# researchaccelerator-hub/distributed-crawler

Measured on AMD Instinct MI355X. Metric: posts/sec (whole node) synthetic feed, higher is better.
Workload: dtype uint8; 1 GPU; model=telegram-crawl 1k-channels x 10k-posts per GPU (BASELINE config #2, weak-scaled), global_batch=1250000, seq_len=0, platform=telegram, parallelism=dp1, channels_per_gpu=1000, posts_per_channel=10000, chunk_posts=1250000, new_discoveries=998486, sink=pinned, pinned=True, max_comments_per_post=3

## Files before the change

crawler_amd/ops/csrc/parse_encode.hip:

```cpp

#include "common.h"
#include "tg_lits.h"

namespace crawl {

#define MAX_LINKS 8
#define TG_STAGE_BYTES 3968

struct BatchView {
  const long* __restrict__ chat_id;
  const long* __restrict__ msg_id;
  const long* __restrict__ text_off;
  const int* __restrict__ date;
  const int* __restrict__ content_type;
  const int* __restrict__ views;
  const int* __restrict__ forwards;
  const int* __restrict__ media_album_id;
  const int* __restrict__ channel_idx;
  const int* __restrict__ flags;
  const int* __restrict__ text_len;
  const int* __restrict__ aux_off;
  const int* __restrict__ aux_len;
  const int* __restrict__ ent_off;
  const int* __restrict__ ent_cnt;
  const int* __restrict__ react_off;
  const int* __restrict__ react_cnt;
  const int* __restrict__ com_off;
  const int* __restrict__ com_cnt;
  const int* __restrict__ poster_off;
  const int* __restrict__ poster_len;
  const unsigned char* __restrict__ pool;
  const int* __restrict__ entities;
  const int* __restrict__ react_emoji;
  const int* __restrict__ react_count;
  const int* __restrict__ com_text_off;
  const int* __restrict__ com_text_len;
  const int* __restrict__ com_handle_off;
  const int* __restrict__ com_handle_len;
  const int* __restrict__ com_views;
  const int* __restrict__ com_replies;
  const int* __restrict__ com_react_off;
  const int* __restrict__ com_react_cnt;
  const long* __restrict__ ch_chat_id;
  const int* __restrict__ ch_member;
  const int* __restrict__ ch_postcount;
  const int* __restrict__ ch_totalviews;
  const int* __restrict__ ch_user_off;
  const int* __restrict__ ch_user_len;
  const int* __restrict__ ch_title_off;
  const int* __restrict__ ch_title_len;
  const unsigned char* __restrict__ emoji_pool;
  const int* __restrict__ emoji_off;
  const int* __restrict__ emoji_len;
  const unsigned char* __restrict__ created_str;
  int created_len;
  const unsigned char* __restrict__ capture_str;
  int capture_len;
  int n;
  int skip_media;
  long min_post_date;
  const unsigned char* __restrict__ ctname_pool;
  const int* __restrict__ ctname_off;
  const int* __restrict__ ctname_len;
};

struct LinkOut {
  unsigned char* __restrict__ name;
  unsigned char* __restrict__ name_len;
  unsigned char* __restrict__ src;
  int* __restrict__ cnt;
  unsigned long long* __restrict__ hash;
};


DEV void utf16_to_bytes(const unsigned char* s, int n, int off16, int len16,
                        int* out_start, int* out_end) {
  int lane = lane_id();
  int run = 0;
  int start = -1, end = -1;
  const int t1 = off16, t2 = off16 + len16;
  for (int base = 0; base < n; base += WAVE) {
    int p = base + lane;
    int u = (p < n) ? u16_units_of_byte(s[p]) : 0;
    int pre = run + wave_prefix_excl(u);
    bool boundary = (p < n) && u > 0;
    unsigned long long m1 = __ballot(boundary && pre == t1);
    unsigned long long m2 = __ballot(boundary && pre == t2);
    if (start < 0 && m1) start = base + __ffsll(m1) - 1;
    if (end < 0 && m2) end = base + __ffsll(m2) - 1;
    run += wave_sum(u);
    if (end >= 0) break;
  }
  if (start < 0) { *out_start = 0; *out_end = 0; return; }
  *out_start = start;
  *out_end = (end >= 0) ? end : n;
}


DEV bool is_reserved_path(const unsigned char* name, int n) {
  const char* tbl[10] = {"joinchat", "addlist", "addstickers", "addtheme",
                         "setlanguage", "share", "proxy", "socks", "login",
                         "confirm"};
  const int lens[10] = {8, 7, 11, 8, 11, 5, 5, 5, 5, 7};
  for (int k = 0; k < 10; ++k) {
    if (lens[k] != n) continue;
    bool eq = true;
    for (int j = 0; j < n; ++j) eq &= (name[j] == (unsigned char)tbl[k][j]);
    if (eq) return true;
  }
  return false;
}

DEV int match_name_at(const unsigned char* s, int hi, int q,
                      unsigned char* name, bool* reserved) {
  *reserved = false;
  if (q >= hi || !is_ascii_letter(s[q])) return 0;
  int len = 0;
  while (len < 32 && q + len < hi && is_word_char(s[q + len])) ++len;
  if (len < 5) return 0;
  for (int j = 0; j < len; ++j) name[j] = to_lower(s[q + j]);
  *reserved = is_reserved_path(name, len);
  return len;
}

DEV int find_tme(const unsigned char* s, int from, int hi, int lane) {
  for (int base = from; base + 5 <= hi; base += WAVE) {
    int p = base + lane;
    bool m = (p + 5 <= hi) && s[p] == 't' && s[p + 1] == '.' &&
             s[p + 2] == 'm' && s[p + 3] == 'e' && s[p + 4] == '/';
    unsigned long long bal = __ballot(m);
    if (bal) return base + __ffsll(bal) - 1;
  }
  return -1;
}

DEV int find_username(const unsigned char* s, int lo, int hi, int lane,
                      unsigned char* name) {
  for (int base = lo; base < hi; base += WAVE) {
    int p = base + lane;
    bool m = false;
    if (p < hi && p + 5 <= hi && is_ascii_letter(s[p])) {
      m = is_word_char(s[p + 1]) && is_word_char(s[p + 2]) &&
          is_word_char(s[p + 3]) && is_word_char(s[p + 4]);
    }
    unsigned long long bal = __ballot(m);
    if (bal) {
      int q = base + __ffsll(bal) - 1;
      int len = 0;
      while (len < 32 && q + len < hi && is_word_char(s[q + len])) ++len;
      for (int j = 0; j < len; ++j) name[j] = to_lower(s[q + j]);
      return len;
    }
  }
  return 0;
}

struct LinkList {
  unsigned char* names;
  unsigned char* lens;
  unsigned char* srcs;
  unsigned long long* hashes;
  int cnt;

  DEV void add(const unsigned char* name, int len, int src, int lane) {
    for (int k = 0; k < cnt; ++k) {
      if (lens[k] != (unsigned char)len) continue;
      bool eq = true;
      for (int j = 0; j < len; ++j) eq &= (names[k * 32 + j] == name[j]);
      if (eq) return;
    }
    if (cnt >= MAX_LINKS) return;
    if (lane == 0) {
      for (int j = 0; j < len; ++j) names[cnt * 32 + j] = name[j];
      lens[cnt] = (unsigned char)len;
      srcs[cnt] = (unsigned char)src;
      hashes[cnt] = fnv1a64(name, len);
    }
    ++cnt;
  }
};

DEV void extract_links(const BatchView& B, int i, LinkList& L, int lane) {
  int ct = B.content_type[i];
  if (ct > 6) return;
  const unsigned char* text = B.pool + B.text_off[i];
  const int tn = B.text_len[i];
  unsigned char name[32];

  const int e0 = B.ent_off[i], ec = B.ent_cnt[i];
  for (int e = e0; e < e0 + ec; ++e) {
    const int* row = B.entities + (long)e * 5;
    int etype = row[0];
    if (etype == 1) {
      const unsigned char* url = B.pool + row[3];
      int un = row[4];
      for (int from = 0;;) {
        int p = find_tme(url, from, un, lane);
        if (p < 0) break;
        bool rsv;
        int len = match_name_at(url, un, p + 5, name, &rsv);
        if (len) {
          if (!rsv) L.add(name, len, 1, lane);
          break;
        }
        from = p + 1;
      }
    } else {
      int lo, hi;
      utf16_to_bytes(text, tn, row[1], row[2], &lo, &hi);
      if (!(lo < hi && hi <= tn)) continue;
      if (etype == 0) {
        int len = find_username(text, lo, hi, lane, name);
        if (len) L.add(name, len, 0, lane);
      } else {
        for (int from = lo;;) {
          int p = find_tme(text, from, hi, lane);
          if (p < 0) break;
          bool rsv;
          int len = match_name_at(text, hi, p + 5, name, &rsv);
          if (len) {
            if (!rsv) L.add(name, len, 2, lane);
            break;
          }
          from = p + 1;
        }
      }
    }
  }

  int cursor = 0;
  int from = 0;
  while (true) {
    int p = find_tme(text, from, tn, lane);
    if (p < 0) break;
    from = p + 1;
    if (p < cursor) continue;
    bool rsv;
    int len = match_name_at(text, tn, p + 5, name, &rsv);
    if (len) {
      if (!rsv) L.add(name, len, 3, lane);
      cursor = p + 5 + len;
      from = cursor;
    }
  }
}


template <bool W>
struct Emit : JsonEmit<W> {
  DEV void qesc(const unsigned char* s, int n) {
    LIT(*this, "\"");
    this->esc(s, n);
    LIT(*this, "\"");
  }
};

struct StagedTabs {
  const unsigned char* emoji_pool;
  const int* emoji_off;
  const int* emoji_len;
  const unsigned char* created;
  const unsigned char* capture;
  const unsigned char* ctname_pool;
  const int* ctname_off;
  const int* ctname_len;
};

template <bool W, bool STAGED>
DEV int emit_line(const BatchView& B, int i, unsigned char* out,
                  LinkList& L, const unsigned char* lds_lits,
                  unsigned char* lds_stage, const StagedTabs* T) {
  const int lane = lane_id();
  Emit<W> e{};
  e.out = out;
  e.cur = 0;
  e.lds = lds_lits;
  const int c = B.channel_idx[i];
  const unsigned char* user = B.pool + B.ch_user_off[c];
  const int user_n = B.ch_user_len[c];
  const unsigned char* title = B.pool + B.ch_title_off[c];
  const int title_n = B.ch_title_len[c];
  const long pub_id = B.msg_id[i] >> 20;
  const int ct = B.content_type[i];
  const int ncom = B.com_cnt[i];
  const bool has_user = user_n > 0;
  const long chat_id_v = B.chat_id[i];
  const int media_album = B.media_album_id[i];
  const int date_v = B.date[i];
  const int views_v = B.views[i];
  const int forwards_v = B.forwards[i];
  const int ch_member_v = B.ch_member[c];
  const int ch_postcount_v = B.ch_postcount[c];
  const int ch_totalviews_v = B.ch_totalviews[c];
  const int flags_v = B.flags[i];
  const int com0_v = B.com_off[i];
  const int react0_v = B.react_off[i];
  const int reactc_v = B.react_cnt[i];
  const int poster_off_v = B.poster_off[i];
  const int poster_len_v = B.poster_len[i];
  const int text_off_v = B.text_off[i];
  const int text_len_v = B.text_len[i];
  const int aux_off_v = B.aux_off[i];
  const int aux_len_v = B.aux_len[i];
  const int ctname_off_v = B.ctname_off[ct];
  const int ctname_len_v = B.ctname_len[ct];
  const unsigned char* desc_p;
  int desc_n;
  if (ct == 0 || ct == 1 || ct == 2 || ct == 4 || ct == 14) {
    desc_p = B.pool + text_off_v;
    desc_n = text_len_v;
  } else if (ct == 3 || ct == 9 || ct == 10 || ct == 11) {
    desc_p = B.pool + aux_off_v;
    desc_n = aux_len_v;
  } else {
    desc_p = nullptr;
    desc_n = 0;
  }
  const unsigned char* poster_p = B.pool + poster_off_v;
  const int* re_src = B.react_emoji + react0_v;
  const int* rcnt_src = B.react_count + react0_v;
  const unsigned char* lnames_src = L.names;
  const unsigned char* llens_src = L.lens;
  if (STAGED) {
    int stage_o = 0;
    auto staged = [&](const unsigned char* ptr,
                      int n) -> const unsigned char* {
      unsigned char* dst = lds_stage + stage_o;
      stage_o += n;
      for (int j = lane; j < n; j += WAVE) dst[j] = ptr[j];
      return dst;
    };
    user = staged(user, user_n);
    title = staged(title, title_n);
    poster_p = staged(poster_p, poster_len_v);
    desc_p = staged(desc_p, desc_n);
    lnames_src = staged(L.names, L.cnt * 32);
    llens_src = staged(L.lens, L.cnt);
    stage_o = (stage_o + 3) & ~3;
    int* s_re = (int*)(lds_stage + stage_o);
    stage_o += reactc_v * 4;
    int* s_rc = (int*)(lds_stage + stage_o);
    stage_o += reactc_v * 4;
    for (int j = lane; j < reactc_v; j += WAVE) {
      s_re[j] = B.react_emoji[react0_v + j];
      s_rc[j] = B.react_count[react0_v + j];
    }
    re_src = s_re;
    rcnt_src = s_rc;
  }
  const unsigned char* emoji_pool_s = STAGED ? T->emoji_pool : B.emoji_pool;
  const int* emoji_off_s = STAGED ? T->emoji_off : B.emoji_off;
  const int* emoji_len_s = STAGED ? T->emoji_len : B.emoji_len;
  const unsigned char* created_s = STAGED ? T->created : B.created_str;
  const unsigned char* capture_s = STAGED ? T->capture : B.capture_str;
  const unsigned char* ctpool_s = STAGED ? T->ctname_pool : B.ctname_pool;

  auto post_link = [&]() {
    if (!has_user) { LIT(e, "\"\""); return; }
    TGLIT(e, TGL_0);
    e.esc(user, user_n);
    LIT(e, "/");
    e.i64(pub_id);
    if (media_album != 0) TGLIT(e, TGL_1);
    LIT(e, "\"");
  };

  TGLIT(e, TGL_2);
  post_link();
  TGLIT(e, TGL_3);
  e.i64(chat_id_v);
  TGLIT(e, TGL_4);
  e.i64(pub_id);
  LIT(e, "-");
  e.esc(user, user_n);
  TGLIT(e, TGL_5);
  post_link();
  TGLIT(e, TGL_6);
  e.rfc3339(date_v);
  TGLIT(e, TGL_7);
  e.raw(created_s, B.created_len);
  TGLIT(e, TGL_8);
  e.i64(views_v);
  TGLIT(e, TGL_9);
  e.i64(views_v);
  TGLIT(e, TGL_10);
  e.i64(forwards_v);
  TGLIT(e, TGL_11);
  e.i64(ncom);
  TGLIT(e, TGL_12);
  e.qesc(title, title_n);
  TGLIT(e, TGL_13);
  e.i64(chat_id_v);
  TGLIT(e, TGL_14);
  e.qesc(title, title_n);
  TGLIT(e, TGL_15);
  e.i64(ch_member_v);
  TGLIT(e, TGL_16);
  e.i64(ch_postcount_v);
  TGLIT(e, TGL_17);
  e.i64(ch_totalviews_v);
  TGLIT(e, TGL_18);
  e.esc(user, user_n);
  TGLIT(e, TGL_19);
  e.esc(user, user_n);
  TGLIT(e, TGL_20);
  e.qesc(desc_p, desc_n);
  TGLIT(e, TGL_21);
  e.raw(ctpool_s + (STAGED ? T->ctname_off[ct] : ctname_off_v),
        STAGED ? T->ctname_len[ct] : ctname_len_v);
  TGLIT(e, TGL_22);
  e.i64(forwards_v);
  TGLIT(e, TGL_23);
  e.i64(ncom);
  TGLIT(e, TGL_17);
  e.i64(views_v);
  TGLIT(e, TGL_24);
  TGLIT(e, TGL_25);
  if ((ct == 3 || ct == 8) && (flags_v & 2)) {
    LIT(e, "AgAD");
    e.i64(pub_id);
    LIT(e, "v");
  }
  TGLIT(e, TGL_26);
  {
    const int c0 = com0_v;
    for (int k = 0; k < ncom; ++k) {
      if (k) LIT(e, ",");
      const int cc = c0 + k;
      TGLIT(e, TGL_27);
      e.qesc(B.pool + B.com_text_off[cc], B.com_text_len[cc]);
      TGLIT(e, TGL_28);
      const int r0 = B.com_react_off[cc], rc = B.com_react_cnt[cc];
      for (int r = 0; r < rc; ++r) {
        if (r) LIT(e, ",");
        int em = B.react_emoji[r0 + r];
        LIT(e, "\"");
        e.raw(emoji_pool_s + emoji_off_s[em], emoji_len_s[em]);
        LIT(e, "\":");
        e.i64(B.react_count[r0 + r]);
      }
      TGLIT(e, TGL_29);
      e.i64(B.com_views[cc]);
      TGLIT(e, TGL_30);
      e.i64(B.com_replies[cc]);
      TGLIT(e, TGL_31);
      e.qesc(B.pool + B.com_handle_off[cc], B.com_handle_len[cc]);
      LIT(e, "}");
    }
  }
  TGLIT(e, TGL_32);
  {
    const int rc = reactc_v;
    for (int r = 0; r < rc; ++r) {
      if (r) LIT(e, ",");
      int em = re_src[r];
      LIT(e, "\"");
      e.raw(emoji_pool_s + emoji_off_s[em], emoji_len_s[em]);
      LIT(e, "\":");
      e.i64(rcnt_src[r]);
    }
  }
  TGLIT(e, TGL_33);
  for (int k = 0; k < L.cnt; ++k) {
    if (k) LIT(e, ",");
    LIT(e, "\"");
    e.raw(lnames_src + k * 32, llens_src[k]);
    LIT(e, "\"");
  }
  TGLIT(e, TGL_34);
  e.raw(capture_s, B.capture_len);
  TGLIT(e, TGL_35);
  e.qesc(poster_p, poster_len_v);
  LIT(e, "}\n");
  return e.cur;
}


__global__ void __launch_bounds__(256, 6)
measure_extract_kernel(BatchView B, LinkOut LO, int* __restrict__ line_len) {
  __shared__ unsigned char s_lits[TG_POOL_BYTES];
  __shared__ unsigned char s_ln[4][MAX_LINKS * 32];
  __shared__ unsigned char s_ll[4][MAX_LINKS];
  __shared__ unsigned char s_ls[4][MAX_LINKS];
  __shared__ unsigned long long s_lh[4][MAX_LINKS];
  for (int t = threadIdx.x; t < TG_POOL_BYTES; t += blockDim.x)
    s_lits[t] = (unsigned char)tg_lit_pool.v[t];
  __syncthreads();
  const int lane = lane_id();
  const int wave = wave_id();
  const int waves_per_grid = gridDim.x * 4;
  for (int i = blockIdx.x * 4 + wave; i < B.n; i += waves_per_grid) {
    if ((long)B.date[i] < B.min_post_date) {
      if (lane == 0) { line_len[i] = 0; LO.cnt[i] = 0; }
      continue;
    }
    LinkList L{&s_ln[wave][0], &s_ll[wave][0], &s_ls[wave][0],
               &s_lh[wave][0], 0};
    extract_links(B, i, L, lane);
    int len = emit_line<false, false>(B, i, nullptr, L, s_lits,
                                     nullptr, nullptr);
    const int nb = L.cnt * 32;
    unsigned char* gname = LO.name + (size_t)i * MAX_LINKS * 32;
    for (int j = lane; j < nb; j += WAVE) gname[j] = s_ln[wave][j];
    if (lane < L.cnt) {
      LO.name_len[(size_t)i * MAX_LINKS + lane] = s_ll[wave][lane];
      LO.src[(size_t)i * MAX_LINKS + lane] = s_ls[wave][lane];
      LO.hash[(size_t)i * MAX_LINKS + lane] = s_lh[wave][lane];
    }
    if (lane == 0) {
      line_len[i] = len;
      LO.cnt[i] = L.cnt;
    }
  }
}

__global__ void __launch_bounds__(256, 4)
write_kernel(BatchView B, LinkOut LO, const long* __restrict__ line_off,
             const int* __restrict__ line_len, unsigned char* __restrict__ out) {
  __shared__ unsigned char s_lits[TG_POOL_BYTES];
  for (int t = threadIdx.x; t < TG_POOL_BYTES; t += blockDim.x)
    s_lits[t] = (unsigned char)tg_lit_pool.v[t];
  __syncthreads();
  const int lane = lane_id();
  const int wave = wave_id();
  const int waves_per_grid = gridDim.x * 4;
  for (int i = blockIdx.x * 4 + wave; i < B.n; i += waves_per_grid) {
    if (line_len[i] == 0) continue;
    LinkList L{LO.name + (size_t)i * MAX_LINKS * 32,
               LO.name_len + (size_t)i * MAX_LINKS,
               LO.src + (size_t)i * MAX_LINKS,
               LO.hash + (size_t)i * MAX_LINKS, LO.cnt[i]};
    emit_line<true, false>(B, i, out + line_off[i], L, s_lits, nullptr,
                           nullptr);
  }
}

#define TG_EMOJI_POOL_CAP 512
#define TG_EMOJI_CAP 64
#define TG_TS_CAP 64
#define TG_CTNAME_POOL_CAP 512
#define TG_CTNAME_CAP 32

__global__ void __launch_bounds__(256, 4)
write_staged_kernel(BatchView B, LinkOut LO, const long* __restrict__ line_off,
                    const int* __restrict__ line_len,
                    unsigned char* __restrict__ out,
                    int n_emoji, int emoji_pool_bytes,
                    int n_ctnames, int ctname_pool_bytes) {
  __shared__ unsigned char s_lits[TG_POOL_BYTES];
  __shared__ unsigned char s_stage[4][TG_STAGE_BYTES];
  __shared__ unsigned char s_emoji_pool[TG_EMOJI_POOL_CAP];
  __shared__ int s_emoji_off[TG_EMOJI_CAP];
  __shared__ int s_emoji_len[TG_EMOJI_CAP];
  __shared__ unsigned char s_created[TG_TS_CAP];
  __shared__ unsigned char s_capture[TG_TS_CAP];
  __shared__ unsigned char s_ctpool[TG_CTNAME_POOL_CAP];
  __shared__ int s_ctoff[TG_CTNAME_CAP];
  __shared__ int s_ctlen[TG_CTNAME_CAP];
  for (int t = threadIdx.x; t < TG_POOL_BYTES; t += blockDim.x)
    s_lits[t] = (unsigned char)tg_lit_pool.v[t];
  for (int t = threadIdx.x; t < emoji_pool_bytes; t += blockDim.x)
    s_emoji_pool[t] = B.emoji_pool[t];
  for (int t = threadIdx.x; t < n_emoji; t += blockDim.x) {
    s_emoji_off[t] = B.emoji_off[t];
    s_emoji_len[t] = B.emoji_len[t];
  }
  for (int t = threadIdx.x; t < B.created_len; t += blockDim.x)
    s_created[t] = B.created_str[t];
  for (int t = threadIdx.x; t < B.capture_len; t += blockDim.x)
    s_capture[t] = B.capture_str[t];
  for (int t = threadIdx.x; t < ctname_pool_bytes; t += blockDim.x)
    s_ctpool[t] = B.ctname_pool[t];
  for (int t = threadIdx.x; t < n_ctnames; t += blockDim.x) {
    s_ctoff[t] = B.ctname_off[t];
    s_ctlen[t] = B.ctname_len[t];
  }
  __syncthreads();
  StagedTabs T{s_emoji_pool, s_emoji_off, s_emoji_len, s_created,
               s_capture, s_ctpool, s_ctoff, s_ctlen};
  const int lane = lane_id();
  const int wave = wave_id();
  const int waves_per_grid = gridDim.x * 4;
  for (int i = blockIdx.x * 4 + wave; i < B.n; i += waves_per_grid) {
    if (line_len[i] == 0) continue;
    LinkList L{LO.name + (size_t)i * MAX_LINKS * 32,
               LO.name_len + (size_t)i * MAX_LINKS,
               LO.src + (size_t)i * MAX_LINKS,
               LO.hash + (size_t)i * MAX_LINKS, LO.cnt[i]};
    emit_line<true, true>(B, i, out + line_off[i], L, s_lits,
                          &s_stage[wave][0], &T);
  }
}


#define LDS_LINE_BYTES 3072

DEV void copy_line(const unsigned char* src, unsigned char* dst, int n,
                   int lane);

__global__ void __launch_bounds__(256)
write_lds_kernel(BatchView B, LinkOut LO, const long* __restrict__ line_off,
                 const int* __restrict__ line_len, unsigned char* __restrict__ out) {
  __shared__ unsigned char lbuf[4][LDS_LINE_BYTES];
  __shared__ unsigned char s_lits[TG_POOL_BYTES];
  for (int t = threadIdx.x; t < TG_POOL_BYTES; t += blockDim.x)
    s_lits[t] = (unsigned char)tg_lit_pool.v[t];
  __syncthreads();
  const int lane = lane_id();
  const int wave = wave_id();
  const int waves_per_grid = gridDim.x * 4;
  for (int i = blockIdx.x * 4 + wave; i < B.n; i += waves_per_grid) {
    const int len = line_len[i];
    if (len == 0) continue;
    LinkList L{LO.name + (size_t)i * MAX_LINKS * 32,
               LO.name_len + (size_t)i * MAX_LINKS,
               LO.src + (size_t)i * MAX_LINKS,
               LO.hash + (size_t)i * MAX_LINKS, LO.cnt[i]};
    if (len > LDS_LINE_BYTES) {
      emit_line<true, false>(B, i, out + line_off[i], L, s_lits,
                             nullptr, nullptr);
      continue;
    }
    emit_line<true, false>(B, i, &lbuf[wave][0], L, s_lits, nullptr,
                           nullptr);
    copy_line(&lbuf[wave][0], out + line_off[i], len, lane);
  }
}


__global__ void __launch_bounds__(256)
write_scratch_kernel(BatchView B, LinkOut LO, unsigned char* __restrict__ scratch,
                     long stride, int* __restrict__ line_len, int* __restrict__ overflow) {
  __shared__ unsigned char s_lits[TG_POOL_BYTES];
  for (int t = threadIdx.x; t < TG_POOL_BYTES; t += blockDim.x)
    s_lits[t] = (unsigned char)tg_lit_pool.v[t];
  __syncthreads();
  const int lane = lane_id();
  const int wave = wave_id();
  const int waves_per_grid = gridDim.x * 4;
  for (int i = blockIdx.x * 4 + wave; i < B.n; i += waves_per_grid) {
    if ((long)B.date[i] < B.min_post_date) {
      if (lane == 0) { line_len[i] = 0; LO.cnt[i] = 0; }
      continue;
    }
    LinkList L{LO.name + (size_t)i * MAX_LINKS * 32,
               LO.name_len + (size_t)i * MAX_LINKS,
               LO.src + (size_t)i * MAX_LINKS,
               LO.hash + (size_t)i * MAX_LINKS, 0};
    extract_links(B, i, L, lane);
    int len = emit_line<true, false>(B, i, scratch + (size_t)i * stride, L,
                                     s_lits, nullptr, nullptr);
    if (lane == 0) {
      line_len[i] = len;
      LO.cnt[i] = L.cnt;
      if (len > stride) atomicMax(overflow, len);
    }
  }
}

DEV void copy_line(const unsigned char* src, unsigned char* dst, int n,
                   int lane) {
  int h = (int)((4 - ((unsigned long)(size_t)dst & 3)) & 3);
  if (h > n) h = n;
  if (lane == 0)
    for (int j = 0; j < h; ++j) dst[j] = src[j];
  const unsigned char* s = src + h;
  unsigned char* d = dst + h;
  int rem = n - h;
  int nw = rem >> 2;
  int sh = (int)((unsigned long)(size_t)s & 3);
  const unsigned int* sw = (const unsigned int*)(s - sh);
  for (int k = lane; k < nw; k += WAVE) {
    unsigned int w0 = sw[k];
    unsigned int v;
    if (sh) {
      unsigned int w1 = sw[k + 1];
      v = (unsigned int)((((unsigned long long)w1 << 32) | w0) >> (8 * sh));
    } else {
      v = w0;
    }
    ((unsigned int*)d)[k] = v;
  }
  if (lane == 0)
    for (int j = h + (nw << 2); j < n; ++j) dst[j] = src[j];
}

__global__ void __launch_bounds__(256)
compact_kernel(const unsigned char* scratch, long stride,
               const long* line_off, const int* line_len,
               unsigned char* out, int n) {
  const int lane = lane_id();
  const int wave = wave_id();
  const int waves_per_grid = gridDim.x * 4;
  for (int i = blockIdx.x * 4 + wave; i < n; i += waves_per_grid) {
    int len = line_len[i];
    if (len == 0) continue;
    copy_line(scratch + (size_t)i * stride, out + line_off[i], len, lane);
  }
}

}


namespace crawl {

static BatchView make_view(void** p, const long* s) {
  BatchView B;
  int k = 0;
  B.chat_id = (const long*)p[k++];
  B.msg_id = (const long*)p[k++];
  B.text_off = (const long*)p[k++];
  B.date = (const int*)p[k++];
  B.content_type = (const int*)p[k++];
  B.views = (const int*)p[k++];
  B.forwards = (const int*)p[k++];
  B.media_album_id = (const int*)p[k++];
  B.channel_idx = (const int*)p[k++];
  B.flags = (const int*)p[k++];
  B.text_len = (const int*)p[k++];
  B.aux_off = (const int*)p[k++];
  B.aux_len = (const int*)p[k++];
  B.ent_off = (const int*)p[k++];
  B.ent_cnt = (const int*)p[k++];
  B.react_off = (const int*)p[k++];
  B.react_cnt = (const int*)p[k++];
  B.com_off = (const int*)p[k++];
  B.com_cnt = (const int*)p[k++];
  B.poster_off = (const int*)p[k++];
  B.poster_len = (const int*)p[k++];
  B.pool = (const unsigned char*)p[k++];
  B.entities = (const int*)p[k++];
  B.react_emoji = (const int*)p[k++];
  B.react_count = (const int*)p[k++];
  B.com_text_off = (const int*)p[k++];
  B.com_text_len = (const int*)p[k++];
  B.com_handle_off = (const int*)p[k++];
  B.com_handle_len = (const int*)p[k++];
  B.com_views = (const int*)p[k++];
  B.com_replies = (const int*)p[k++];
  B.com_react_off = (const int*)p[k++];
  B.com_react_cnt = (const int*)p[k++];
  B.ch_chat_id = (const long*)p[k++];
  B.ch_member = (const int*)p[k++];
  B.ch_postcount = (const int*)p[k++];
  B.ch_totalviews = (const int*)p[k++];
  B.ch_user_off = (const int*)p[k++];
  B.ch_user_len = (const int*)p[k++];
  B.ch_title_off = (const int*)p[k++];
  B.ch_title_len = (const int*)p[k++];
  B.emoji_pool = (const unsigned char*)p[k++];
  B.emoji_off = (const int*)p[k++];
  B.emoji_len = (const int*)p[k++];
  B.created_str = (const unsigned char*)p[k++];
  B.capture_str = (const unsigned char*)p[k++];
  B.ctname_pool = (const unsigned char*)p[k++];
  B.ctname_off = (const int*)p[k++];
  B.ctname_len = (const int*)p[k++];
  B.n = (int)s[0];
  B.skip_media = (int)s[1];
  B.min_post_date = s[2];
  B.created_len = (int)s[3];
  B.capture_len = (int)s[4];
  return B;
}

static LinkOut make_links(void** p) {
  LinkOut L;
  L.name = (unsigned char*)p[0];
  L.name_len = (unsigned char*)p[1];
  L.src = (unsigned char*)p[2];
  L.cnt = (int*)p[3];
  L.hash = (unsigned long long*)p[4];
  return L;
}

}

extern "C" {

int crawl_batch_ptr_count() { return 49; }

int crawl_measure_extract(void** batch_ptrs, const long* scalars,
                          void** link_ptrs, void* line_len, int grid,
                          void* stream) {
  crawl::BatchView B = crawl::make_view(batch_ptrs, scalars);
  crawl::LinkOut LO = crawl::make_links(link_ptrs);
  hipLaunchKernelGGL(crawl::measure_extract_kernel, dim3(grid), dim3(256), 0,
                     (hipStream_t)stream, B, LO, (int*)line_len);
  return (int)hipGetLastError();
}

int crawl_write(void** batch_ptrs, const long* scalars, void** link_ptrs,
                const void* line_off, const void* line_len, void* out,
                int grid, void* stream) {
  crawl::BatchView B = crawl::make_view(batch_ptrs, scalars);
  crawl::LinkOut LO = crawl::make_links(link_ptrs);
  hipLaunchKernelGGL(crawl::write_kernel, dim3(grid), dim3(256), 0,
                     (hipStream_t)stream, B, LO, (const long*)line_off,
                     (const int*)line_len, (unsigned char*)out);
  return (int)hipGetLastError();
}

int crawl_write_staged(void** batch_ptrs, const long* scalars,
                       void** link_ptrs, const void* line_off,
                       const void* line_len, void* out,
                       int n_emoji, int emoji_pool_bytes,
                       int n_ctnames, int ctname_pool_bytes,
                       int grid, void* stream) {
  crawl::BatchView B = crawl::make_view(batch_ptrs, scalars);
  crawl::LinkOut LO = crawl::make_links(link_ptrs);
  hipLaunchKernelGGL(crawl::write_staged_kernel, dim3(grid), dim3(256), 0,
                     (hipStream_t)stream, B, LO, (const long*)line_off,
                     (const int*)line_len, (unsigned char*)out,
                     n_emoji, emoji_pool_bytes, n_ctnames,
                     ctname_pool_bytes);
  return (int)hipGetLastError();
}

int crawl_stage_budget() { return TG_STAGE_BYTES; }

int crawl_write_scratch(void** batch_ptrs, const long* scalars,
                        void** link_ptrs, void* scratch, long stride,
                        void* line_len, void* overflow, int grid,
                        void* stream) {
  crawl::BatchView B = crawl::make_view(batch_ptrs, scalars);
  crawl::LinkOut LO = crawl::make_links(link_ptrs);
  hipLaunchKernelGGL(crawl::write_scratch_kernel, dim3(grid), dim3(256), 0,
                     (hipStream_t)stream, B, LO, (unsigned char*)scratch,
                     stride, (int*)line_len, (int*)overflow);
  return (int)hipGetLastError();
}

int crawl_write_lds(void** batch_ptrs, const long* scalars, void** link_ptrs,
                    const void* line_off, const void* line_len, void* out,
                    int grid, void* stream) {
  crawl::BatchView B = crawl::make_view(batch_ptrs, scalars);
  crawl::LinkOut LO = crawl::make_links(link_ptrs);
  hipLaunchKernelGGL(crawl::write_lds_kernel, dim3(grid), dim3(256), 0,
                     (hipStream_t)stream, B, LO, (const long*)line_off,
                     (const int*)line_len, (unsigned char*)out);
  return (int)hipGetLastError();
}

int crawl_compact(const void* scratch, long stride, const void* line_off,
                  const void* line_len, void* out, int n, int grid,
                  void* stream) {
  hipLaunchKernelGGL(crawl::compact_kernel, dim3(grid), dim3(256), 0,
                     (hipStream_t)stream, (const unsigned char*)scratch,
                     stride, (const long*)line_off, (const int*)line_len,
                     (unsigned char*)out, n);
  return (int)hipGetLastError();
}

}
```

crawler_amd/ops/gpu.py:

```python
from __future__ import annotations

import ctypes
import dataclasses
import datetime as _dt
import os
from typing import List, Optional, Tuple

import torch

from ..models.post import format_go_time
from . import batch as B

_CSRC = os.path.dirname(os.path.abspath(__file__)) + "/csrc"
_LIB_PATH = os.path.join(_CSRC, "libcrawlhip.so")

MAX_LINKS = 8

_BATCH_PTR_ORDER = [
    "chat_id", "msg_id", "text_off",
    "m:date", "m:content_type", "m:views", "m:forwards", "m:media_album_id",
    "m:channel_idx", "m:flags", "m:text_len", "m:aux_off", "m:aux_len",
    "m:ent_off", "m:ent_cnt", "m:react_off", "m:react_cnt", "m:com_off",
    "m:com_cnt", "m:poster_off", "m:poster_len",
    "text_pool", "entities", "react_emoji", "react_count",
    "com_text_off", "com_text_len", "com_handle_off", "com_handle_len",
    "com_views", "com_replies", "com_react_off", "com_react_cnt",
    "ch_chat_id", "ch_member", "ch_postcount", "ch_totalviews",
    "ch_user_off", "ch_user_len", "ch_title_off", "ch_title_len",
]

_lib = None


def lib_available() -> bool:
    return os.path.exists(_LIB_PATH)


def load_lib():
    global _lib
    if _lib is not None:
        return _lib
    lib = ctypes.CDLL(_LIB_PATH)
    lib.crawl_batch_ptr_count.restype = ctypes.c_int
    lib.crawl_measure_extract.restype = ctypes.c_int
    lib.crawl_measure_extract.argtypes = [
        ctypes.POINTER(ctypes.c_void_p), ctypes.POINTER(ctypes.c_long),
        ctypes.POINTER(ctypes.c_void_p), ctypes.c_void_p, ctypes.c_int,
        ctypes.c_void_p,
    ]
    lib.crawl_write.restype = ctypes.c_int
    lib.crawl_write.argtypes = [
        ctypes.POINTER(ctypes.c_void_p), ctypes.POINTER(ctypes.c_long),
        ctypes.POINTER(ctypes.c_void_p), ctypes.c_void_p, ctypes.c_void_p,
        ctypes.c_void_p, ctypes.c_int, ctypes.c_void_p,
    ]
    lib.crawl_write_staged.restype = ctypes.c_int
    lib.crawl_write_staged.argtypes = [
        ctypes.POINTER(ctypes.c_void_p), ctypes.POINTER(ctypes.c_long),
        ctypes.POINTER(ctypes.c_void_p), ctypes.c_void_p, ctypes.c_void_p,
        ctypes.c_void_p, ctypes.c_int, ctypes.c_int, ctypes.c_int,
        ctypes.c_int, ctypes.c_int, ctypes.c_void_p,
    ]
    lib.crawl_stage_budget.restype = ctypes.c_int
    _bind_dedup(lib)
    _bind_feedgen(lib)
    _bind_v2(lib)
    _bind_yt(lib)
    _bind_aux(lib)
    _lib = lib
    return lib


def _bind_v2(lib):
    lib.crawl_write_lds.restype = ctypes.c_int
    lib.crawl_write_lds.argtypes = [
        ctypes.POINTER(ctypes.c_void_p), ctypes.POINTER(ctypes.c_long),
        ctypes.POINTER(ctypes.c_void_p), ctypes.c_void_p, ctypes.c_void_p,
        ctypes.c_void_p, ctypes.c_int, ctypes.c_void_p,
    ]
    lib.crawl_write_scratch.restype = ctypes.c_int
    lib.crawl_write_scratch.argtypes = [
        ctypes.POINTER(ctypes.c_void_p), ctypes.POINTER(ctypes.c_long),
        ctypes.POINTER(ctypes.c_void_p), ctypes.c_void_p, ctypes.c_long,
        ctypes.c_void_p, ctypes.c_void_p, ctypes.c_int, ctypes.c_void_p,
    ]
    lib.crawl_compact.restype = ctypes.c_int
    lib.crawl_compact.argtypes = [
        ctypes.c_void_p, ctypes.c_long, ctypes.c_void_p, ctypes.c_void_p,
        ctypes.c_void_p, ctypes.c_int, ctypes.c_int, ctypes.c_void_p,
    ]


def _bind_yt(lib):
    for fn in ("crawl_yt_gen_meta", "crawl_yt_gen_fill",
               "crawl_yt_gen_channels"):
        getattr(lib, fn).restype = ctypes.c_int
    lib.crawl_yt_gen_meta.argtypes = (
        [ctypes.c_longlong] * 5 + [ctypes.c_void_p] * 11
        + [ctypes.c_void_p])
    lib.crawl_yt_gen_fill.argtypes = (
        [ctypes.c_longlong] * 5 + [ctypes.c_void_p] * 6
        + [ctypes.c_void_p])
    lib.crawl_yt_gen_channels.argtypes = (
        [ctypes.c_longlong] * 3 + [ctypes.c_void_p, ctypes.c_longlong]
        + [ctypes.c_void_p] * 9 + [ctypes.c_void_p])
    lib.crawl_yt_ptr_count.restype = ctypes.c_int
    lib.crawl_yt_measure.restype = ctypes.c_int
    lib.crawl_yt_measure.argtypes = [
        ctypes.POINTER(ctypes.c_void_p), ctypes.POINTER(ctypes.c_long),
        ctypes.c_void_p, ctypes.c_int, ctypes.c_void_p,
    ]
    lib.crawl_yt_write.restype = ctypes.c_int
    lib.crawl_yt_write.argtypes = [
        ctypes.POINTER(ctypes.c_void_p), ctypes.POINTER(ctypes.c_long),
        ctypes.c_void_p, ctypes.c_void_p, ctypes.c_int, ctypes.c_void_p,
    ]


_YT_PTR_ORDER = [
    "vid_off", "channel_idx", "published", "views", "likes", "comments",
    "duration_s", "lang", "title_off", "title_len", "desc_off", "desc_len",
    "pool", "ch_id_off", "ch_title_off", "ch_title_len", "ch_desc_off",
    "ch_desc_len", "ch_subs", "ch_videos", "ch_views", "ch_country_off",
    "ch_country_len", "ch_published",
]


def yt_parse_encode(batch, now: Optional[_dt.datetime] = None,
                    grid: int = 0) -> Tuple[torch.Tensor, torch.Tensor,
                                            torch.Tensor]:
    lib = require_lib()
    dev = batch.device
    assert dev.type == "cuda"
    n = batch.n
    now = now or _dt.datetime.now(_dt.timezone.utc)
    created = format_go_time(now.replace(microsecond=0)).encode()
    capture = format_go_time(now).encode()
    to_dev = lambda b: torch.frombuffer(bytearray(b or b"\0"),
                                        dtype=torch.uint8).to(dev)
    label_t = to_dev(batch.crawl_label.encode())
    from ..youtube.batch import LANGS

    lang_t = to_dev("".join(LANGS).encode())
    created_t, capture_t = to_dev(created), to_dev(capture)
    tensors = [getattr(batch, name) for name in _YT_PTR_ORDER]
    tensors += [label_t, lang_t, created_t, capture_t]
    ptrs = _ptr_array(tensors)
    assert len(tensors) == lib.crawl_yt_ptr_count()
    scalars = (ctypes.c_long * 4)(
        n, len(batch.crawl_label.encode()), len(created), len(capture)
    )
    if grid <= 0:
        grid = min((n + 3) // 4, 8192)
    stream_ptr = ctypes.c_void_p(torch.cuda.current_stream().cuda_stream)
    line_len = torch.zeros(n, dtype=torch.int32, device=dev)
    rc = lib.crawl_yt_measure(ptrs, scalars,
                              ctypes.c_void_p(line_len.data_ptr()),
                              grid, stream_ptr)
    if rc != 0:
        raise RuntimeError(f"crawl_yt_measure failed: hip {rc}")
    line_off = torch.zeros(n, dtype=torch.int64, device=dev)
    torch.cumsum(line_len.to(torch.int64)[:-1], 0, out=line_off[1:])
    total = int(line_off[-1].item() + line_len[-1].item()) if n else 0
    out = torch.empty(total, dtype=torch.uint8, device=dev)
    rc = lib.crawl_yt_write(ptrs, scalars,
                            ctypes.c_void_p(line_off.data_ptr()),
                            ctypes.c_void_p(out.data_ptr()),
                            grid, stream_ptr)
    if rc != 0:
        raise RuntimeError(f"crawl_yt_write failed: hip {rc}")
    return out, line_off, line_len




def _bind_aux(lib):
    lib.crawl_channel_stats.restype = ctypes.c_int
    lib.crawl_channel_stats.argtypes = [ctypes.c_void_p] * 4 + [
        ctypes.c_int, ctypes.c_int] + [ctypes.c_void_p] * 5 + [
        ctypes.c_void_p]
    lib.crawl_reservoir_sample.restype = ctypes.c_int
    lib.crawl_reservoir_sample.argtypes = [
        ctypes.c_long, ctypes.c_int, ctypes.c_int, ctypes.c_int,
        ctypes.c_void_p, ctypes.c_int, ctypes.c_void_p,
    ]
    lib.crawl_html_classify.restype = ctypes.c_int
    lib.crawl_html_classify.argtypes = [
        ctypes.c_void_p, ctypes.c_void_p, ctypes.c_void_p, ctypes.c_int,
        ctypes.c_void_p, ctypes.c_void_p, ctypes.c_int, ctypes.c_void_p,
    ]


def channel_stats(batch: B.MessageBatch, line_len=None):
    lib = require_lib()
    dev = batch.device
    K = batch.n_channels
    P = batch.n // K
    assert K * P == batch.n, "batch must be K x P channel-grouped"
    out = {
        "views": torch.zeros(K, dtype=torch.int64, device=dev),
        "forwards": torch.zeros(K, dtype=torch.int64, device=dev),
        "replies": torch.zeros(K, dtype=torch.int64, device=dev),
        "posts": torch.zeros(K, dtype=torch.int32, device=dev),
        "totals": torch.zeros(4, dtype=torch.int64, device=dev),
    }
    m = batch.meta
    rc = lib.crawl_channel_stats(
        ctypes.c_void_p(m["views"].data_ptr()),
        ctypes.c_void_p(m["forwards"].data_ptr()),
        ctypes.c_void_p(m["reply_count"].data_ptr()),
        ctypes.c_void_p(line_len.data_ptr()) if line_len is not None
        else None,
        P, K,
        ctypes.c_void_p(out["views"].data_ptr()),
        ctypes.c_void_p(out["forwards"].data_ptr()),
        ctypes.c_void_p(out["replies"].data_ptr()),
        ctypes.c_void_p(out["posts"].data_ptr()),
        ctypes.c_void_p(out["totals"].data_ptr()),
        ctypes.c_void_p(torch.cuda.current_stream().cuda_stream),
    )
    if rc != 0:
        raise RuntimeError(f"crawl_channel_stats failed: hip {rc}")
    return out


def reservoir_sample(batch: B.MessageBatch, k: int, seed: int = 0):
    lib = require_lib()
    dev = batch.device
    K = batch.n_channels
    P = batch.n // K
    out = torch.zeros((K, k), dtype=torch.int32, device=dev)
    rc = lib.crawl_reservoir_sample(
        seed, P, K, k, ctypes.c_void_p(out.data_ptr()),
        min(max(1, (K + 3) // 4), 8192),
        ctypes.c_void_p(torch.cuda.current_stream().cuda_stream),
    )
    if rc != 0:
        raise RuntimeError(f"crawl_reservoir_sample failed: hip {rc}")
    return out


def reservoir_sample_oracle(P: int, K: int, k: int, seed: int = 0):
    def sm64(x):
        z = (x + 0x9E3779B97F4A7C15) & (2**64 - 1)
        z = ((z ^ (z >> 30)) * 0xBF58476D1CE4E5B9) & (2**64 - 1)
        z = ((z ^ (z >> 27)) * 0x94D049BB133111EB) & (2**64 - 1)
        return z ^ (z >> 31)

    out = []
    for c in range(K):
        slot = list(range(c * P, c * P + k))
        for i in range(k, P):
            r = sm64((seed ^ ((c * 0x9E3779B1 + i) & (2**64 - 1)))
                     & (2**64 - 1))
            j = r % (i + 1)
            if j < k:
                slot[j] = c * P + i
        out.append(slot)
    return out


_HTML_STATUS = ["valid", "not_channel", "invalid"]
_HTML_REASON = ["", "not_supergroup", "not_found", "not_found",
                "unrecognized"]


def html_classify(docs, device="cuda:0"):
    lib = require_lib()
    dev = torch.device(device)
    n = len(docs)
    blob = b"".join(docs) or b"\0"
    pool = torch.frombuffer(bytearray(blob), dtype=torch.uint8).to(dev)
    offs, cur = [], 0
    lens = []
    for d in docs:
        offs.append(cur)
        lens.append(len(d))
        cur += len(d)
    doc_off = torch.tensor(offs, dtype=torch.int64, device=dev)
    doc_len = torch.tensor(lens, dtype=torch.int32, device=dev)
    status = torch.zeros(n, dtype=torch.int32, device=dev)
    reason = torch.zeros(n, dtype=torch.int32, device=dev)
    rc = lib.crawl_html_classify(
        ctypes.c_void_p(pool.data_ptr()),
        ctypes.c_void_p(doc_off.data_ptr()),
        ctypes.c_void_p(doc_len.data_ptr()), n,
        ctypes.c_void_p(status.data_ptr()),
        ctypes.c_void_p(reason.data_ptr()),
        min(max(1, (n + 3) // 4), 8192),
        ctypes.c_void_p(torch.cuda.current_stream().cuda_stream),
    )
    if rc != 0:
        raise RuntimeError(f"crawl_html_classify failed: hip {rc}")
    st = status.cpu().numpy()
    rs = reason.cpu().numpy()
    return [(_HTML_STATUS[int(st[i])], _HTML_REASON[int(rs[i])])
            for i in range(n)]


def _bind_dedup(lib):
    lib.crawl_claim_links.restype = ctypes.c_int
    lib.crawl_claim_links.argtypes = [
        ctypes.c_void_p, ctypes.c_void_p, ctypes.c_int, ctypes.c_int,
        ctypes.c_void_p, ctypes.c_longlong, ctypes.c_void_p, ctypes.c_void_p,
        ctypes.c_int, ctypes.c_void_p,
    ]
    lib.crawl_bloom_update.restype = ctypes.c_int
    lib.crawl_bloom_update.argtypes = [
        ctypes.c_void_p, ctypes.c_void_p, ctypes.c_int, ctypes.c_int,
        ctypes.c_void_p, ctypes.c_longlong, ctypes.c_int, ctypes.c_void_p,
    ]
    lib.crawl_insert_hashes.restype = ctypes.c_int
    lib.crawl_insert_hashes.argtypes = [
        ctypes.c_void_p, ctypes.c_long, ctypes.c_void_p, ctypes.c_longlong,
        ctypes.c_int, ctypes.c_void_p,
    ]


def _bind_feedgen(lib):
    lib.crawl_feed_meta.restype = ctypes.c_int
    lib.crawl_feed_meta.argtypes = [
        ctypes.POINTER(ctypes.c_void_p), ctypes.POINTER(ctypes.c_long),
        ctypes.c_void_p, ctypes.POINTER(ctypes.c_void_p), ctypes.c_int,
        ctypes.c_void_p,
    ]
    lib.crawl_feed_fill.restype = ctypes.c_int
    lib.crawl_feed_fill.argtypes = [
        ctypes.POINTER(ctypes.c_void_p), ctypes.POINTER(ctypes.c_long),
        ctypes.c_void_p, ctypes.c_void_p, ctypes.c_void_p, ctypes.c_void_p,
        ctypes.c_void_p, ctypes.POINTER(ctypes.c_void_p), ctypes.c_int,
        ctypes.c_void_p,
    ]
    lib.crawl_feed_comments.restype = ctypes.c_int
    lib.crawl_feed_comments.argtypes = [
        ctypes.POINTER(ctypes.c_void_p), ctypes.POINTER(ctypes.c_long),
        ctypes.c_void_p, ctypes.c_void_p, ctypes.c_long, ctypes.c_void_p,
        ctypes.c_long, ctypes.c_long, ctypes.POINTER(ctypes.c_void_p),
        ctypes.c_int, ctypes.c_void_p,
    ]


def require_lib():
    if not lib_available():
        raise RuntimeError(
            "libcrawlhip.so not built — run __graft_entry__.build() "
            "(hipcc --offload-arch=gfx950) before GPU execution; the Python "
            "golden path is not a substitute on GPU hosts"
        )
    return load_lib()


def _const_tables(device):
    epool = b"".join(e.encode("utf-8") for e in B.EMOJI_TABLE)
    eoff, cur = [], 0
    elen = []
    for e in B.EMOJI_TABLE:
        n = len(e.encode("utf-8"))
        eoff.append(cur)
        elen.append(n)
        cur += n
    cpool = b"".join(c.encode() for c in B.CONTENT_TYPES)
    coff, ccur = [], 0
    clen = []
    for c in B.CONTENT_TYPES:
        coff.append(ccur)
        clen.append(len(c))
# ... 372 lines not shown
```

Baseline: 27.57 million posts/s.

## Emit post comments lane-parallel with LDS staging and assembly buffers

Comments were previously serialized one at a time, with the whole wave cooperating on each one. They are now handled one per lane. Each lane stages its comment text and handle into a per-wave LDS source buffer, computes the lengths, and uses a wave prefix sum to give each lane its offset. In write mode each lane assembles its comment into an LDS assembly buffer, and the wave then copies the buffer out. Oversized comments fall back to the old wave-cooperative path. The added LDS (about 4x1280 bytes in measure, plus 4x3080 bytes in the write kernels) may reduce occupancy, and the per-lane serial escaping may diverge.

```diff
diff --git a/crawler_amd/ops/csrc/parse_encode.hip b/crawler_amd/ops/csrc/parse_encode.hip
--- a/crawler_amd/ops/csrc/parse_encode.hip
+++ b/crawler_amd/ops/csrc/parse_encode.hip
@@ -266,10 +266,282 @@
   const int* ctname_len;
 };
 
-template <bool W, bool STAGED>
+
+#define TG_COM_LANE_BYTES 128
+#define TG_COM_LANE_REACTS 4
+#ifndef TG_COM_SRC_BYTES
+#define TG_COM_SRC_BYTES 1280
+#endif
+#ifndef TG_COM_ASM_BYTES
+#define TG_COM_ASM_BYTES 3072
+#endif
+#define TG_COM_ASM_PAD 8
+
+DEV void copy_line(const unsigned char* src, unsigned char* dst, int n,
+                   int lane);
+
+struct ComTabs {
+  const unsigned char* pool;
+  const int* text_off;
+  const int* text_len;
+  const int* handle_off;
+  const int* handle_len;
+  const int* views;
+  const int* replies;
+  const int* react_off;
+  const int* react_cnt;
+  const int* react_emoji;
+  const int* react_count;
+  const unsigned char* emoji_pool;
+  const int* emoji_off;
+  const int* emoji_len;
+};
+
+template <bool W>
+DEV void emit_comment_wave(Emit<W>& e, const ComTabs& C, int k, int cc) {
+  if (k) LIT(e, ",");
+  TGLIT(e, TGL_27);
+  e.qesc(C.pool + C.text_off[cc], C.text_len[cc]);
+  TGLIT(e, TGL_28);
+  const int r0 = C.react_off[cc], rc = C.react_cnt[cc];
+  for (int r = 0; r < rc; ++r) {
+    if (r) LIT(e, ",");
+    int em = C.react_emoji[r0 + r];
+    LIT(e, "\"");
+    e.raw(C.emoji_pool + C.emoji_off[em], C.emoji_len[em]);
+    LIT(e, "\":");
+    e.i64(C.react_count[r0 + r]);
+  }
+  TGLIT(e, TGL_29);
+  e.i64(C.views[cc]);
+  TGLIT(e, TGL_30);
+  e.i64(C.replies[cc]);
+  TGLIT(e, TGL_31);
+  e.qesc(C.pool + C.handle_off[cc], C.handle_len[cc]);
+  LIT(e, "}");
+}
+
+DEV void lane_stage(const unsigned char* g, int n, unsigned char* slot) {
+  unsigned* dw = (unsigned*)slot;
+  const int nd = n >> 2;
+  for (int d = 0; d < nd; d += 4) {
+    unsigned w[4];
+#pragma unroll
+    for (int j = 0; j < 4; ++j)
+      if (d + j < nd) __builtin_memcpy(&w[j], g + 4 * (d + j), 4);
+#pragma unroll
+    for (int j = 0; j < 4; ++j)
+      if (d + j < nd) dw[d + j] = w[j];
+  }
+  if (n & 3) {
+    unsigned t = 0;
+    for (int j = 0; j < (n & 3); ++j)
+      t |= (unsigned)g[4 * nd + j] << (8 * j);
+    dw[nd] = t;
+  }
+}
+
+template <bool WR, int ID>
+DEV int lane_lit(const unsigned char* lits, unsigned char* d) {
+  constexpr int N = tg_lit_lens[ID];
+  if (WR) {
+    const unsigned char* s = lits + tg_lit_off(ID);
+#pragma unroll
+    for (int k = 0; k + 4 <= N; k += 4) {
+      unsigned w;
+      __builtin_memcpy(&w, s + k, 4);
+      __builtin_memcpy(d + k, &w, 4);
+    }
+#pragma unroll
+    for (int k = N & ~3; k < N; ++k) d[k] = s[k];
+  }
+  return N;
+}
+
+template <bool WR>
+DEV int lane_chr(unsigned char* d, char c) {
+  if (WR) d[0] = (unsigned char)c;
+  return 1;
+}
+
+template <bool WR>
+DEV int lane_dec(unsigned char* d, int v) {
+  const int n = i64_dec_len((long long)v);
+  if (WR) {
+    unsigned u = v < 0 ? 0u - (unsigned)v : (unsigned)v;
+    if (v < 0) d[0] = '-';
+    for (int k = n - 1; k >= (v < 0 ? 1 : 0); --k) {
+      d[k] = (unsigned char)('0' + u % 10u);
+      u /= 10u;
+    }
+  }
+  return n;
+}
+
+template <bool WR>
+DEV int lane_esc(const unsigned char* s, int n, unsigned char* d) {
+  int o = 0, p = 0;
+  int exact = 0;
+  unsigned pw = 0, w = 0;
+  while (p < n) {
+    if (exact == 0 && p + 4 <= n) {
+      __builtin_memcpy(&w, s + p, 4);
+      const bool risk = (pw >> 24) == 0xE2u || (pw >> 16) == 0x80E2u;
+      pw = w;
+      if (!risk && !JsonEmit<false>::swar_special(w)) {
+        if (WR) __builtin_memcpy(d + o, &w, 4);
+        o += 4;
+        p += 4;
+        continue;
+      }
+      exact = 4;
+    }
+    const int el = escape_len_at(s, n, p);
+    if (WR && el) escape_write_at(s, n, p, d + o);
+    o += el;
+    ++p;
+    if (exact) --exact;
+  }
+  return o;
+}
+
+struct LaneComment {
+  const unsigned char* text;
+  const unsigned char* handle;
+  int text_n, handle_n;
+  int views, replies;
+  int r0, rc;
+  bool comma;
+};
+
+template <bool WR>
+DEV int lane_comment(const LaneComment& c, const ComTabs& C,
+                     const unsigned char* lits, unsigned char* d) {
+  int o = 0;
+  if (c.comma) o += lane_chr<WR>(d + o, ',');
+  o += lane_lit<WR, TGL_27_id>(lits, d + o);
+  o += lane_chr<WR>(d + o, '"');
+  o += lane_esc<WR>(c.text, c.text_n, d + o);
+  o += lane_chr<WR>(d + o, '"');
+  o += lane_lit<WR, TGL_28_id>(lits, d + o);
+  for (int r = 0; r < c.rc; ++r) {
+    if (r) o += lane_chr<WR>(d + o, ',');
+    const int em = C.react_emoji[c.r0 + r];
+    const int en = C.emoji_len[em];
+    o += lane_chr<WR>(d + o, '"');
+    if (WR) {
+      const unsigned char* ep = C.emoji_pool + C.emoji_off[em];
+      for (int j = 0; j < en; ++j) d[o + j] = ep[j];
+    }
+    o += en;
+    o += lane_chr<WR>(d + o, '"');
+    o += lane_chr<WR>(d + o, ':');
+    o += lane_dec<WR>(d + o, C.react_count[c.r0 + r]);
+  }
+  o += lane_lit<WR, TGL_29_id>(lits, d + o);
+  o += lane_dec<WR>(d + o, c.views);
+  o += lane_lit<WR, TGL_30_id>(lits, d + o);
+  o += lane_dec<WR>(d + o, c.replies);
+  o += lane_lit<WR, TGL_31_id>(lits, d + o);
+  o += lane_chr<WR>(d + o, '"');
+  o += lane_esc<WR>(c.handle, c.handle_n, d + o);
+  o += lane_chr<WR>(d + o, '"');
+  o += lane_chr<WR>(d + o, '}');
+  return o;
+}
+
+template <bool W>
+DEV void emit_comments(Emit<W>& e, const ComTabs& C, int c0, int ncom,
+                       unsigned char* com_src, unsigned char* com_asm) {
+  const int lane = lane_id();
+  int zero = 0;
+  asm volatile("" : "+v"(c0), "+v"(ncom), "+v"(zero));
+  c0 = __builtin_amdgcn_readfirstlane(c0);
+  ncom = __builtin_amdgcn_readfirstlane(ncom);
+  zero = __builtin_amdgcn_readfirstlane(zero);
+  com_src += zero;
+  com_asm += zero;
+  int k0 = 0;
+  bool alone = false;
+  while (k0 < ncom) {
+    if (alone) {
+      emit_comment_wave<W>(e, C, k0, c0 + k0);
+      alone = false;
+      k0 += 1;
+      continue;
+    }
+    const bool in = lane < ncom - k0;
+    const int cc = c0 + k0 + lane;
+    int to = 0, tl = 0, ho = 0, hl = 0, vw = 0, rp = 0, r0 = 0, rc = 0;
+    if (in) {
+      to = C.text_off[cc];
+      tl = C.text_len[cc];
+      ho = C.handle_off[cc];
+      hl = C.handle_len[cc];
+      vw = C.views[cc];
+      rp = C.replies[cc];
+      r0 = C.react_off[cc];
+      rc = C.react_cnt[cc];
+    }
+    const bool big = tl < 0 || hl < 0 || rc < 0 ||
+                     tl + hl > TG_COM_LANE_BYTES || rc > TG_COM_LANE_REACTS;
+    const int tslot = (tl + 3) & ~3;
+    const int slot = (in && !big) ? tslot + ((hl + 3) & ~3) : 0;
+    const int sp = wave_prefix_excl(slot);
+    const bool ok = in && !big && sp + slot <= TG_COM_SRC_BYTES;
+    const unsigned long long bad = __ballot(!ok);
+    const int g = bad ? __ffsll(bad) - 1 : WAVE;
+    if (g == 0) {
+      alone = true;
+      continue;
+    }
+    LaneComment c{com_src + sp, com_src + sp + tslot, tl, hl, vw, rp,
+                  r0, rc, k0 + lane > 0};
+    int len = 0;
+    if (lane < g) {
+      lane_stage(C.pool + to, tl, com_src + sp);
+      lane_stage(C.pool + ho, hl, com_src + sp + tslot);
+      len = lane_comment<false>(c, C, nullptr, nullptr);
+    }
+    if (!W) {
+      e.cur += wave_sum(len);
+      k0 += g;
+      continue;
+    }
+    const int ep = wave_prefix_excl(len);
+    int a = 0;
+    while (a < g) {
+      const int base = __builtin_amdgcn_readlane(ep, a);
+      const bool fits = lane >= a && lane < g &&
+                        ep + len - base <= TG_COM_ASM_BYTES;
+      const int cnt = __popcll(__ballot(fits));
+      if (cnt == 0) {
+        alone = true;
+        break;
+      }
+      if (fits)
+        lane_comment<true>(c, C, e.lds, com_asm + (ep - base));
+      const int bytes =
+          __builtin_amdgcn_readlane(ep + len, a + cnt - 1) - base;
+      __builtin_amdgcn_fence(__ATOMIC_RELEASE, "wavefront");
+      __builtin_amdgcn_wave_barrier();
+      __builtin_amdgcn_fence(__ATOMIC_ACQUIRE, "wavefront");
+      copy_line(com_asm, e.out + e.cur, bytes, lane);
+      __builtin_amdgcn_fence(__ATOMIC_RELEASE, "wavefront");
+      __builtin_amdgcn_wave_barrier();
+      __builtin_amdgcn_fence(__ATOMIC_ACQUIRE, "wavefront");
+      e.cur += bytes;
+      a += cnt;
+    }
+    k0 += a;
+  }
+}
+
+template <bool W, bool STAGED, bool GROUPED>
 DEV int emit_line(const BatchView& B, int i, unsigned char* out,
                   LinkList& L, const unsigned char* lds_lits,
-                  unsigned char* lds_stage, const StagedTabs* T) {
+                  unsigned char* lds_stage, const StagedTabs* T,
+                  unsigned char* com_src, unsigned char* com_asm) {
   const int lane = lane_id();
   Emit<W> e{};
   e.out = out;
@@ -422,31 +694,23 @@
     LIT(e, "v");
   }
   TGLIT(e, TGL_26);
-  {
-    const int c0 = com0_v;
-    for (int k = 0; k < ncom; ++k) {
-      if (k) LIT(e, ",");
-      const int cc = c0 + k;
-      TGLIT(e, TGL_27);
-      e.qesc(B.pool + B.com_text_off[cc], B.com_text_len[cc]);
-      TGLIT(e, TGL_28);
-      const int r0 = B.com_react_off[cc], rc = B.com_react_cnt[cc];
-      for (int r = 0; r < rc; ++r) {
-        if (r) LIT(e, ",");
-        int em = B.react_emoji[r0 + r];
-        LIT(e, "\"");
-        e.raw(emoji_pool_s + emoji_off_s[em], emoji_len_s[em]);
-        LIT(e, "\":");
-        e.i64(B.react_count[r0 + r]);
-      }
-      TGLIT(e, TGL_29);
-      e.i64(B.com_views[cc]);
-      TGLIT(e, TGL_30);
-      e.i64(B.com_replies[cc]);
-      TGLIT(e, TGL_31);
-      e.qesc(B.pool + B.com_handle_off[cc], B.com_handle_len[cc]);
-      LIT(e, "}");
-    }
+  if constexpr (GROUPED) {
+    if (__builtin_expect(ncom > 0, 0)) {
+      const ComTabs C{B.pool, B.com_text_off, B.com_text_len,
+                      B.com_handle_off, B.com_handle_len, B.com_views,
+                      B.com_replies, B.com_react_off, B.com_react_cnt,
+                      B.react_emoji, B.react_count, emoji_pool_s,
+                      emoji_off_s, emoji_len_s};
+      emit_comments<W>(e, C, com0_v, ncom, com_src, com_asm);
+    }
+  } else {
+    const ComTabs C{B.pool, B.com_text_off, B.com_text_len,
+                    B.com_handle_off, B.com_handle_len, B.com_views,
+                    B.com_replies, B.com_react_off, B.com_react_cnt,
+                    B.react_emoji, B.react_count, emoji_pool_s,
+                    emoji_off_s, emoji_len_s};
+    for (int k = 0; k < ncom; ++k)
+      emit_comment_wave<W>(e, C, k, com0_v + k);
   }
   TGLIT(e, TGL_32);
   {
@@ -483,6 +747,7 @@
   __shared__ unsigned char s_ll[4][MAX_LINKS];
   __shared__ unsigned char s_ls[4][MAX_LINKS];
   __shared__ unsigned long long s_lh[4][MAX_LINKS];
+  __shared__ __align__(16) unsigned char s_csrc[4][TG_COM_SRC_BYTES];
   for (int t = threadIdx.x; t < TG_POOL_BYTES; t += blockDim.x)
     s_lits[t] = (unsigned char)tg_lit_pool.v[t];
   __syncthreads();
@@ -497,8 +762,9 @@
     LinkList L{&s_ln[wave][0], &s_ll[wave][0], &s_ls[wave][0],
                &s_lh[wave][0], 0};
     extract_links(B, i, L, lane);
-    int len = emit_line<false, false>(B, i, nullptr, L, s_lits,
-                                     nullptr, nullptr);
+    int len = emit_line<false, false, true>(B, i, nullptr, L, s_lits,
+                                           nullptr, nullptr,
+                                           &s_csrc[wave][0], nullptr);
     const int nb = L.cnt * 32;
     unsigned char* gname = LO.name + (size_t)i * MAX_LINKS * 32;
     for (int j = lane; j < nb; j += WAVE) gname[j] = s_ln[wave][j];
@@ -518,6 +784,9 @@
 write_kernel(BatchView B, LinkOut LO, const long* __restrict__ line_off,
              const int* __restrict__ line_len, unsigned char* __restrict__ out) {
   __shared__ unsigned char s_lits[TG_POOL_BYTES];
+  __shared__ __align__(16) unsigned char s_csrc[4][TG_COM_SRC_BYTES];
+  __shared__ __align__(16) unsigned char
+      s_casm[4][TG_COM_ASM_BYTES + TG_COM_ASM_PAD];
   for (int t = threadIdx.x; t < TG_POOL_BYTES; t += blockDim.x)
     s_lits[t] = (unsigned char)tg_lit_pool.v[t];
   __syncthreads();
@@ -530,8 +799,9 @@
                LO.name_len + (size_t)i * MAX_LINKS,
                LO.src + (size_t)i * MAX_LINKS,
                LO.hash + (size_t)i * MAX_LINKS, LO.cnt[i]};
-    emit_line<true, false>(B, i, out + line_off[i], L, s_lits, nullptr,
-                           nullptr);
+    emit_line<true, false, true>(B, i, out + line_off[i], L, s_lits,
+                                 nullptr, nullptr, &s_csrc[wave][0],
+                                 &s_casm[wave][0]);
   }
 }
 
@@ -557,6 +827,9 @@
   __shared__ unsigned char s_ctpool[TG_CTNAME_POOL_CAP];
   __shared__ int s_ctoff[TG_CTNAME_CAP];
   __shared__ int s_ctlen[TG_CTNAME_CAP];
+  __shared__ __align__(16) unsigned char s_csrc[4][TG_COM_SRC_BYTES];
+  __shared__ __align__(16) unsigned char
+      s_casm[4][TG_COM_ASM_BYTES + TG_COM_ASM_PAD];
   for (int t = threadIdx.x; t < TG_POOL_BYTES; t += blockDim.x)
     s_lits[t] = (unsigned char)tg_lit_pool.v[t];
   for (int t = threadIdx.x; t < emoji_pool_bytes; t += blockDim.x)
@@ -587,8 +860,9 @@
                LO.name_len + (size_t)i * MAX_LINKS,
                LO.src + (size_t)i * MAX_LINKS,
                LO.hash + (size_t)i * MAX_LINKS, LO.cnt[i]};
-    emit_line<true, true>(B, i, out + line_off[i], L, s_lits,
-                          &s_stage[wave][0], &T);
+    emit_line<true, true, true>(B, i, out + line_off[i], L, s_lits,
+                                &s_stage[wave][0], &T, &s_csrc[wave][0],
+                                &s_casm[wave][0]);
   }
 }
 
@@ -617,12 +891,12 @@
                LO.src + (size_t)i * MAX_LINKS,
                LO.hash + (size_t)i * MAX_LINKS, LO.cnt[i]};
     if (len > LDS_LINE_BYTES) {
-      emit_line<true, false>(B, i, out + line_off[i], L, s_lits,
-                             nullptr, nullptr);
+      emit_line<true, false, false>(B, i, out + line_off[i], L, s_lits,
+                                    nullptr, nullptr, nullptr, nullptr);
       continue;
     }
-    emit_line<true, false>(B, i, &lbuf[wave][0], L, s_lits, nullptr,
-                           nullptr);
+    emit_line<true, false, false>(B, i, &lbuf[wave][0], L, s_lits,
+                                  nullptr, nullptr, nullptr, nullptr);
     copy_line(&lbuf[wave][0], out + line_off[i], len, lane);
   }
 }
@@ -648,8 +922,9 @@
                LO.src + (size_t)i * MAX_LINKS,
                LO.hash + (size_t)i * MAX_LINKS, 0};
     extract_links(B, i, L, lane);
-    int len = emit_line<true, false>(B, i, scratch + (size_t)i * stride, L,
-                                     s_lits, nullptr, nullptr);
+    int len = emit_line<true, false, false>(
+        B, i, scratch + (size_t)i * stride, L, s_lits, nullptr, nullptr,
+        nullptr, nullptr);
     if (lane == 0) {
       line_len[i] = len;
       LO.cnt[i] = L.cnt;
@@ -819,6 +1094,10 @@
 
 int crawl_stage_budget() { return TG_STAGE_BYTES; }
 
+int crawl_comment_lane_limit() { return TG_COM_LANE_BYTES; }
+int crawl_comment_react_limit() { return TG_COM_LANE_REACTS; }
+int crawl_comment_asm_bytes() { return TG_COM_ASM_BYTES; }
+
 int crawl_write_scratch(void** batch_ptrs, const long* scalars,
                         void** link_ptrs, void* scratch, long stride,
                         void* line_len, void* overflow, int grid,
diff --git a/crawler_amd/ops/gpu.py b/crawler_amd/ops/gpu.py
--- a/crawler_amd/ops/gpu.py
+++ b/crawler_amd/ops/gpu.py
@@ -62,6 +62,9 @@
         ctypes.c_int, ctypes.c_int, ctypes.c_void_p,
     ]
     lib.crawl_stage_budget.restype = ctypes.c_int
+    for fn in ("crawl_comment_lane_limit", "crawl_comment_react_limit",
+               "crawl_comment_asm_bytes"):
+        getattr(lib, fn).restype = ctypes.c_int
     _bind_dedup(lib)
     _bind_feedgen(lib)
     _bind_v2(lib)
```

Result: no change. 27.27 million posts/s (median of 2 runs) (-1.1%).
